# second-state/qwen3_asr_rs

Measured on NVIDIA H100. Metric: real-time factor (audio-sec/wall-sec) Qwen3-ASR-0.6B 30s clips, higher is better.
Workload: dtype f32 (bf16 weights, fp32-exact activations)

## Files before the change

### qwen3_asr_rs_b200/csrc/decode_mega.cu

```cuda
#include "mega_common.cuh"

namespace asrb {

namespace mega {

struct Params {
    const DecLayerW* layers;
    const bf16* lm_head;
    const bf16* embed;
    const float* final_norm;
    const float* rope_cos; const float* rope_sin;
    float eps;
    int L, H, QD, KVD, I, V, nq, nkv, group;
    float* x;
    float* kcache; float* vcache; size_t cache_layer_stride; int max_ctx;
    int nsplit;
    float* part_val; int* part_idx;
    int* pos; int* done; int* next_id; int* ids_out; int* n_out; int max_new;
    unsigned* bar;
    uint2* qkv_ll; uint2* part_ll;
    uint32_t* sx;
    long long* dbg;
    float* part_sum;
    float* lp_out;
    float* eos_lp;
    float* tk_part_val; int* tk_part_idx;
    int* tk_ids; float* tk_lp;
    int* tk_eos_ids; float* tk_eos_lp;
    const SampleParams* smp;
    int row;
    float* part_max; float* part_sel;
    uint32_t* rep_bits;
    int rep_words;
    const RepParams* rep;
};

static_assert(KV_KEYS * HD * 4 == SLOT_BYTES, "K / V tiles travel through the weight ring: one tile per slot");

template <int K>
__device__ __forceinline__ void load_xr(const float* xs, float (&xr)[K / 32], int lane) {
    const int sw = ((lane >> 2) & 1) * 4;
#pragma unroll
    for (int c = 0; c < K / 256; ++c) {
        const float4 a = *reinterpret_cast<const float4*>(xs + (c * 32 + lane) * 8 + sw);
        const float4 b = *reinterpret_cast<const float4*>(xs + (c * 32 + lane) * 8 + 4 - sw);
        xr[c * 8 + 0] = a.x; xr[c * 8 + 1] = a.y; xr[c * 8 + 2] = a.z; xr[c * 8 + 3] = a.w;
        xr[c * 8 + 4] = b.x; xr[c * 8 + 5] = b.y; xr[c * 8 + 6] = b.z; xr[c * 8 + 7] = b.w;
    }
}
// ... 78 lines not shown
        d0 = fmaf(bf16_lo(wd.F), X0, d0); d1 = fmaf(bf16_hi(wd.F), X1, d1);
        ROW4_STEP(x, xr[c * 8 + 0], xr[c * 8 + 1])
        ROW4_STEP(y, xr[c * 8 + 2], xr[c * 8 + 3])
        ROW4_STEP(z, xr[c * 8 + 4], xr[c * 8 + 5])
        ROW4_STEP(w, xr[c * 8 + 6], xr[c * 8 + 7])
#undef ROW4_STEP
    }
    const float ra = a0 + a1, rb = b0 + b1, rc = c0 + c1, rd = d0 + d1;
    const bool h16 = lane & 16, h8 = lane & 8;
    float k0 = (h16 ? rc : ra) + __shfl_xor_sync(0xffffffffu, h16 ? ra : rc, 16);
    float k1 = (h16 ? rd : rb) + __shfl_xor_sync(0xffffffffu, h16 ? rb : rd, 16);
    float keep = (h8 ? k1 : k0) + __shfl_xor_sync(0xffffffffu, h8 ? k0 : k1, 8);
#pragma unroll
    for (int o = 4; o > 0; o >>= 1) keep += __shfl_xor_sync(0xffffffffu, keep, o);
    return keep;
}

__device__ __forceinline__ float warp_reduce8(const float (&a)[8], int lane) {
    const bool h16 = lane & 16, h8 = lane & 8, h4 = lane & 4;
    float k[4];
#pragma unroll
    for (int i = 0; i < 4; ++i) k[i] = (h16 ? a[4 + i] : a[i]) + __shfl_xor_sync(0xffffffffu, h16 ? a[i] : a[4 + i], 16);
    float m0 = (h8 ? k[2] : k[0]) + __shfl_xor_sync(0xffffffffu, h8 ? k[0] : k[2], 8);
    float m1 = (h8 ? k[3] : k[1]) + __shfl_xor_sync(0xffffffffu, h8 ? k[1] : k[3], 8);
    float v = (h4 ? m1 : m0) + __shfl_xor_sync(0xffffffffu, h4 ? m0 : m1, 4);
    v += __shfl_xor_sync(0xffffffffu, v, 2);
    v += __shfl_xor_sync(0xffffffffu, v, 1);
    return v;
}

// ... 321 lines not shown
    ring.slots = smem;
    ring.nslot = NS;
    float* xs = reinterpret_cast<float*>(smem + (size_t)NS * SLOT_BYTES);
    float* xres = xs + XS_FLOATS;
    float* pbuf = xres + XRES_MAX;
    float* ropes = pbuf + 2 * PARAM_FLOATS;
    DecLayerW* ltab = reinterpret_cast<DecLayerW*>(ropes + 128);
    uint64_t* bars = reinterpret_cast<uint64_t*>(ltab + MAX_LAYERS);
    ring.full = bars; ring.empty = bars + NSLOT_MAX;
    uint64_t* p_full = bars + 2 * NSLOT_MAX; uint64_t* p_empty = p_full + 2;
    float* red = reinterpret_cast<float*>(bars + 2 * NSLOT_MAX + 4);
    int* ired = reinterpret_cast<int*>(red + 64);
    float* part = reinterpret_cast<float*>(ired + 64);
    const int tid = threadIdx.x, lane = tid & 31, warp = tid >> 5;
    const bool is_producer = warp == NCONS_WARPS;

    if (__ldcg(p.done) != 0) return;

    if (tid == 0) {
        for (int i = 0; i < NS; ++i) { mbar_init(&ring.full[i], 1); mbar_init(&ring.empty[i], NCONS_WARPS); }
        for (int i = 0; i < 2; ++i) { mbar_init(&p_full[i], 1); mbar_init(&p_empty[i], NCONS_WARPS); }
        asm volatile("fence.mbarrier_init.release.cluster;" ::: "memory");
    }
    const int pos = __ldcg(p.pos);
    {
        const uint2* src = reinterpret_cast<const uint2*>(p.layers);
        uint2* dst = reinterpret_cast<uint2*>(ltab);
        for (int i = tid; i < p.L * (int)(sizeof(DecLayerW) / 8); i += NTHREADS) dst[i] = src[i];
        if (tid < 64) ropes[tid] = p.rope_cos[(size_t)pos * 64 + tid];
        else if (tid < 128) ropes[tid] = p.rope_sin[(size_t)pos * 64 + tid - 64];
// ... 48 lines not shown
                        bulk_g2s(pb, p.final_norm, H * 4, &p_full[l & 1]);
                        break;
                    }
                }
                const DecLayerW w = ltab[l];
                issue_slice(make_slice(w.wqkv, QD + 2 * p.KVD, H, 1));
                if (n_old > 0) {
                    const size_t off = (size_t)l * p.cache_layer_stride + kv_row;
                    issue(p.kcache + off, (uint32_t)n_old * HD * 4);
                    issue(p.vcache + off, (uint32_t)n_old * HD * 4);
                }
                issue_slice(make_slice(w.wo, H, QD, 1));
                issue_slice(make_slice(w.wgu, 2 * I, H, 2));
                issue_slice(make_slice(w.wdown, H, I, 1));
            }
            issue_slice(make_slice(p.lm_head, p.V, H, 1));
        }
        return;
    }

    long long* dbg_row = nullptr; int dbg_i = 0;
    if (p.dbg && (blockIdx.x == 0 || blockIdx.x == gridDim.x - 1)) dbg_row = p.dbg + (blockIdx.x == 0 ? 0 : DBG_SLOTS);
    MEGA_MARK();
    const int half = HD / 2;
    const float* cs = ropes;
    const float* sn = ropes + half;
    const unsigned G = gridDim.x;
    RepBits rb{};
    if constexpr (REP) {
        const Slice sl = make_slice(nullptr, p.V, H, 1);
        uint32_t* hist = p.rep_bits + (size_t)blockIdx.x * 2 * p.rep_words;
// ... 272 lines not shown
        cons_sync();
        if (lane == 0) mbar_arrive(&p_empty[l & 1]);
    }
    float nrf;
    {
        const float ss = sx_gather<H>(sx_cur + (size_t)(p.L - 1) * SXL + H, xs);
        mbar_wait(&p_full[p.L & 1], (p.L >> 1) & 1);
        nrf = norm_scale(ss, H, p.eps, red);
    }
    static_assert(!(SAMPLE && TOPK), "sampling is never combined with the candidate lists");
    static_assert(4 * NCONS_WARPS <= 62, "per-warp records must fit red / ired");
    constexpr bool SLP = SAMPLE && LOGPROB;
    Draw dr{};
    float smx = -INFINITY, ssel = 0.f;
    if constexpr (SAMPLE) dr = make_draw(p.smp, __ldcg(p.n_out), p.row);
    consume<H, ME_ARGMAX, LOGPROB, TOPK, SAMPLE, REP>(make_slice(p.lm_head, p.V, H, 1), ring, q, xs, nullptr, 0u, nullptr, best_v, best_i,
                                                      best_s, pbuf + (p.L & 1) * PARAM_FLOATS, nrf, nullptr, &tk, &dr, &smx, &ssel, &rb);
    MEGA_MARK();
#pragma unroll
    for (int o = 8; o <= 16; o <<= 1) {
        if constexpr (SAMPLE) {
            sample_merge_xor<LOGPROB>(o, best_v, best_i, best_s, smx, ssel);
        } else {
            const float ov = __shfl_xor_sync(0xffffffffu, best_v, o); const int oi = __shfl_xor_sync(0xffffffffu, best_i, o);
            if constexpr (LOGPROB) best_s = lse_merge(best_v, best_s, ov, __shfl_xor_sync(0xffffffffu, best_s, o));
            if (ov > best_v || (ov == best_v && oi < best_i)) { best_v = ov; best_i = oi; }
            if constexpr (TOPK) tk_merge_xor(tk, o);
        }
    }
    cons_sync();
    float* tkv = xs; int* tki = reinterpret_cast<int*>(xs + NCONS_WARPS * TK_MAX);
    if (lane == 0) { red[warp] = best_v; ired[warp] = best_i; if constexpr (LOGPROB) red[NCONS_WARPS + warp] = best_s; }
// ... 10 lines not shown
            float M = -INFINITY;
            for (int wq = 0; wq < NCONS_WARPS; ++wq) M = fmaxf(M, red[2 * NCONS_WARPS + wq]);
            float sum = 0.f;
            for (int wq = 0; wq < NCONS_WARPS; ++wq) sum += lse_rescale(red[NCONS_WARPS + wq], red[2 * NCONS_WARPS + wq], M);
            p.part_sum[blockIdx.x] = sum; p.part_max[blockIdx.x] = M; p.part_sel[blockIdx.x] = red[3 * NCONS_WARPS + ws];
        }
        else if constexpr (LOGPROB) {
            float sum = 0.f;
            for (int wq = 0; wq < NCONS_WARPS; ++wq) sum += lse_rescale(red[NCONS_WARPS + wq], red[wq], v);
            p.part_sum[blockIdx.x] = sum;
        }
        if constexpr (TOPK) {
            for (int wq = 1; wq < NCONS_WARPS; ++wq) tk_merge_from(tk, tkv + wq * TK_MAX, tki + wq * TK_MAX, false);
            tk_store(tk, p.tk_part_val + (size_t)blockIdx.x * TK_MAX, p.tk_part_idx + (size_t)blockIdx.x * TK_MAX);
        }
        __threadfence();
        unsigned t = atomicAdd(p.bar, 1u);
        is_last = (t == G - 1);
    }
    cons_sync();
    if (!is_last) return;
    __threadfence();
    {
        float v = -INFINITY; int idx = 0x7fffffff;
        int rec = 0; float mloc = -INFINITY;
        for (int i = tid; i < (int)G; i += NCONS) {
            float pv = __ldcg(p.part_val + i); int pi = __ldcg(p.part_idx + i);
            if (pv > v || (pv == v && pi < idx)) { v = pv; idx = pi; if constexpr (SLP) rec = i; }
            if constexpr (SLP) mloc = fmaxf(mloc, __ldcg(p.part_max + i));
        }
// ... 40 lines not shown
                if (red[wq] > v || (red[wq] == v && ired[wq] < idx)) { v = red[wq]; idx = ired[wq]; if constexpr (SLP) rec = ired[NCONS_WARPS + wq]; }
            int tok = idx;
            if constexpr (SLP) lp = (__ldcg(p.part_sel + rec) - M) + lp;
            const int n = *p.n_out;
            if constexpr (LOGPROB) {
                if (tok == 151643 || tok == 151645) *p.eos_lp = lp;
                else if (n < p.max_new) p.lp_out[n] = lp;
            }
            if constexpr (TOPK) {
                if (tok == 151643 || tok == 151645) tk_write(tk, lp, p.tk_eos_ids, p.tk_eos_lp);
                else if (n < p.max_new) tk_write(tk, lp, p.tk_ids + (size_t)n * TK_MAX, p.tk_lp + (size_t)n * TK_MAX);
            }
            if (tok == 151643 || tok == 151645 || n >= p.max_new) { *p.done = 1; *p.next_id = -1; tok = -1; }
            else { p.ids_out[n] = tok; *p.n_out = n + 1; *p.pos = pos + 1; *p.next_id = tok; }
            tok_s = tok;
            p.bar[0] = 0;
            p.bar[1] = p.bar[1] + 1;
            p.bar[3] = p.bar[3] + 1;
        }
        cons_sync();
        const int tok = tok_s;
        if (tok >= 0) {
            const bf16* e = p.embed + (size_t)tok * H;
            for (int i = tid; i < H; i += NCONS) p.x[i] = __bfloat162float(e[i]);
        }
    }
}

}

// ... 11 lines not shown
    return c.hidden_size == H && c.num_attention_heads * c.head_dim == QD && c.intermediate_size == I;
}

bool decode_mega_supported(const Model& m, int B, int ctx) {
    const int max_ctx = ctx;
    const asrb_dims& c = m.d.c;
    if (B < 1 || c.head_dim != 128) return false;
    const int group = c.num_attention_heads / c.num_key_value_heads;
    if (group + 2 > mega::NCONS_WARPS) return false;
    if ((size_t)(group * 128 + 256 + group * mega::KV_KEYS + 8 + mega::NCONS_WARPS * 2 * 128 + mega::NCONS_WARPS * 4 + 8) > (size_t)mega_xs_floats(c.intermediate_size)) return false;
    if (m.ctx->smem_optin < mega_smem_bytes(c.hidden_size, c.intermediate_size, mega_nslot(c))) return false;
    if ((c.hidden_size + m.ctx->sm_count - 1) / m.ctx->sm_count + 1 > mega::XRES_MAX) return false;
    if (c.num_hidden_layers > 32) return false;
    if ((max_ctx + mega::KV_KEYS - 1) / mega::KV_KEYS > mega::MAX_SPLITS) return false;
    if (((max_ctx + mega::KV_KEYS - 1) / mega::KV_KEYS) * c.num_key_value_heads > m.ctx->sm_count) return false;
    return dims_match<1024, 2048, 3072>(c) || dims_match<2048, 2048, 6144>(c) || dims_match<256, 512, 512>(c);
}

size_t decode_mega_part_floats(const Model& m) {
    const asrb_dims& c = m.d.c;
    const int group = c.num_attention_heads / c.num_key_value_heads;
    const size_t words = (size_t)m.d.qkv_dim + (size_t)m.ctx->sm_count * group * mega::PSTRIDE + 64;
    return 2 * words + 64;
}
size_t decode_mega_sx_bytes(const Model& m) {
    const asrb_dims& c = m.d.c;
    return 2 * (size_t)c.num_hidden_layers * (2 * (size_t)c.hidden_size + m.d.q_dim + c.intermediate_size) * sizeof(uint32_t);
}

template <bool LP, bool TK, bool SM, bool RP>
// ... 3 lines not shown
    return (const void*)mega::decode_step_kernel<256, 512, 512, 6, LP, TK, SM, RP>;
}
template <bool RP>
static const void* step_fn(const DecodeBufs& b, const asrb_dims& c) {
    if (b.sample) return b.logprobs ? step_fn_dims<true, false, true, RP>(c) : step_fn_dims<false, false, true, RP>(c);
    if (b.topk) return step_fn_dims<true, true, false, RP>(c);
    if (b.logprobs) return step_fn_dims<true, false, false, RP>(c);
    return step_fn_dims<false, false, false, RP>(c);
}

void launch_decode_step_mega(const Model& m, const DecodeBufs& b, int B, float* kcache, float* vcache,
                             size_t cache_layer_stride, size_t cache_seq_stride, int max_ctx, int ctx_now, const MegaBufs& mb,
                             cudaStream_t st, int64_t* launches) {
    ASRB_REQUIRE(decode_mega_supported(m, B, ctx_now), ASRB_ERR_STATE, "fused decode step not supported for this model/batch/context");
    ASRB_REQUIRE(m.d_dec_layers && mb.bar && mb.part && mb.sx_seq, ASRB_ERR_STATE, "fused decode step buffers missing");
    const asrb_dims& c = m.d.c;
    const int G = m.ctx->sm_count;
    const int group = c.num_attention_heads / c.num_key_value_heads;
    const int nsplit = std::min(mega::MAX_SPLITS, std::min(G / c.num_key_value_heads, (max_ctx + mega::KV_KEYS - 1) / mega::KV_KEYS));
    const size_t smem = mega_smem_bytes(c.hidden_size, c.intermediate_size, mega_nslot(c));
    const void* fn = b.rep ? step_fn<true>(b, c) : step_fn<false>(b, c);
    ASRB_CUDA_CHECK(cudaFuncSetAttribute(fn, cudaFuncAttributeMaxDynamicSharedMemorySize, (int)smem));
    for (int sb = 0; sb < B; ++sb) {
        mega::Params p{};
        p.layers = m.d_dec_layers; p.lm_head = m.lm_head; p.embed = m.embed; p.final_norm = m.final_norm_sw;
        p.rope_cos = m.rope_cos; p.rope_sin = m.rope_sin; p.eps = (float)c.rms_norm_eps;
        p.L = c.num_hidden_layers; p.H = c.hidden_size; p.QD = m.d.q_dim; p.KVD = m.d.kv_dim; p.I = c.intermediate_size;
        p.V = c.vocab_size; p.nq = c.num_attention_heads; p.nkv = c.num_key_value_heads; p.group = group;
        p.x = b.x + (size_t)sb * c.hidden_size;
        p.kcache = kcache + (size_t)sb * cache_seq_stride; p.vcache = vcache + (size_t)sb * cache_seq_stride;
// ... 7 lines not shown
        p.part_ll = w;
        p.sx = mb.sx_seq;
        p.dbg = mb.dbg;
        g_last_dbg = mb.dbg;
        if (b.logprobs) { p.part_sum = b.part_sum; p.lp_out = b.lp_out + (size_t)sb * b.max_new; p.eos_lp = b.eos_lp + sb; }
        if (b.topk) {
            p.tk_part_val = b.tk_part_val; p.tk_part_idx = b.tk_part_idx;
            p.tk_ids = b.tk_ids + (size_t)sb * b.max_new * TK_MAX; p.tk_lp = b.tk_lp + (size_t)sb * b.max_new * TK_MAX;
            p.tk_eos_ids = b.tk_eos_ids + (size_t)sb * TK_MAX; p.tk_eos_lp = b.tk_eos_lp + (size_t)sb * TK_MAX;
        }
        if (b.sample) {
            p.smp = b.smp; p.row = sb;
            if (b.logprobs) { p.part_max = b.part_max; p.part_sel = b.part_sel; }
        }
        if (b.rep) { p.rep_bits = b.rep_mask; p.rep_words = rep_cta_words(c, G); p.rep = b.rep_params; }
        if (mb.steps_issued && ++*mb.steps_issued >= 0xFFFF00u) {
            ASRB_CUDA_CHECK(cudaMemsetAsync(mb.part, 0, mb.part_bytes, st));
            const unsigned one = 1;
            ASRB_CUDA_CHECK(cudaMemcpyAsync(mb.bar + 1, &one, sizeof(one), cudaMemcpyHostToDevice, st));
            *mb.steps_issued = 1;
        }
        void* args[] = {(void*)&p};
        ASRB_CUDA_CHECK(cudaLaunchCooperativeKernel(fn, dim3(G), dim3(mega::NTHREADS), args, smem, st));
        if (launches) *launches += 1;
    }
}

int decode_mega_debug_timeline(long long* out, int cap) {
    if (!g_last_dbg || cap < 2 * mega::DBG_SLOTS) return 0;
    cudaDeviceSynchronize();
// ... 7 lines not shown
```

### qwen3_asr_rs_b200/csrc/internal.h

```cpp
#pragma once
#include <atomic>
#include <map>
#include <string>
#include <vector>
#include "../../include/asr_b200.h"
#include "common.cuh"

namespace asrb {

struct Dims {
    asrb_dims c;
    int enc_hd;
    int chunk_frames;
    int chunks_per_window;
    int conv_h[4];
    int conv_w[4];
    int tok_per_chunk;
    int cpad;
    int feat;
    int q_dim, kv_dim, qkv_dim;
    void derive();
};
void validate_dims(const asrb_dims& d);
inline int conv_out_len(int l) { return (l - 1) / 2 + 1; }
// ... 33 lines not shown
    float *mel_fb = nullptr, *dft_cos = nullptr, *dft_sin = nullptr, *hann = nullptr, *dft_tw = nullptr;
    int* mel_krange = nullptr;
    float *conv1_w = nullptr, *conv1_b = nullptr, *conv2_b = nullptr, *conv3_b = nullptr, *conv_out_b = nullptr;
    bf16 *conv2_w = nullptr, *conv3_w = nullptr, *conv_out_w = nullptr;
    float* pos_emb = nullptr;
    std::vector<EncLayerW> enc;
    float *lnpost_w = nullptr, *lnpost_b = nullptr, *proj1_b = nullptr, *proj2_b = nullptr;
    bf16 *proj1 = nullptr, *proj2 = nullptr;
    bf16 *embed = nullptr, *lm_head = nullptr;
    std::vector<DecLayerW> dec;
    float* final_norm = nullptr;
    DecLayerW* d_dec_layers = nullptr;
    float* final_norm_sw = nullptr;
    DecLayerW* d_dec_layers_b = nullptr;
    bf16* lm_head_b = nullptr;
    float *rope_cos = nullptr, *rope_sin = nullptr;
    int rope_max_pos = 0;

    ~Model();
};

enum { A_PLAIN = 0, A_CONV = 1 };
struct GemmA {
    int mode = A_PLAIN;
    const bf16* a = nullptr;
    size_t plane_stride = 0;
    int nplanes = 3;
    int M = 0, K = 0, lda = 0;
    int OH = 0, OW = 0, Hh = 0, Wh = 0, cpad = 0;
};
// ... 90 lines not shown
    float* part_max;
    float* part_sel;
    bool rep;
    const RepParams* rep_params;
    uint32_t* rep_mask;
    int rep_words;
};
void launch_rep_mask(const DecodeBufs& b, int R, cudaStream_t st, int64_t* launches);
inline int rep_cta_words(const asrb_dims& c, int G) { return ((c.vocab_size + G - 1) / G + 31) / 32 + 1; }
void launch_decode_step_phases(const Model& m, const DecodeBufs& b, int B, float* kcache, float* vcache,
                               size_t cache_layer_stride, size_t cache_seq_stride, int max_ctx,
                               bool write_logits, cudaStream_t st, int64_t* launches);
size_t dec_attn_smem_bytes(const Model& m, int max_ctx);
struct MegaBufs { unsigned* bar = nullptr; float* part = nullptr; long long* dbg = nullptr; size_t part_bytes = 0; unsigned* steps_issued = nullptr;
                  uint32_t* sx = nullptr; size_t sx_bytes = 0; int* sx_nb = nullptr;
                  uint32_t* sx_seq = nullptr; };
size_t decode_mega_part_floats(const Model& m);
size_t decode_mega_sx_bytes(const Model& m);
size_t decode_batch_part_floats(const Model& m);
size_t decode_batch_sx_bytes(const Model& m);
bool decode_batch_supported(const Model& m, int B, int ctx);
int decode_mega_dbg_slots();
void launch_greedy(const Model& m, const DecodeBufs& b, int B, cudaStream_t st, int64_t* launches);
void launch_lmhead_argmax(const Model& m, const float* x_rows, const int* d_row_idx, int B,
                          const DecodeBufs& b, bool write_logits, cudaStream_t st, int64_t* launches);

constexpr int BEAM_MAX = 6;
struct BeamUtt {
    int t;
    int done;
    int S;
    int nfin;
// ... 27 lines not shown
```

### qwen3_asr_rs_b200/csrc/model.cu

```cuda
#include <cmath>
#include <cstring>
#include "internal.h"

namespace asrb {

void Dims::derive() {
    enc_hd = c.d_model / c.encoder_attention_heads;
    chunk_frames = 2 * c.n_window;
    chunks_per_window = c.n_window_infer / chunk_frames;
    conv_h[0] = c.num_mel_bins;
    conv_w[0] = chunk_frames;
    for (int i = 1; i < 4; ++i) { conv_h[i] = conv_out_len(conv_h[i - 1]); conv_w[i] = conv_out_len(conv_w[i - 1]); }
    tok_per_chunk = conv_w[3];
    cpad = ((c.downsample_hidden_size + 63) / 64) * 64;
    feat = c.downsample_hidden_size * conv_h[3];
    q_dim = c.num_attention_heads * c.head_dim;
    kv_dim = c.num_key_value_heads * c.head_dim;
    qkv_dim = q_dim + 2 * kv_dim;
}

Model::~Model() {
    for (auto& kv : raw) if (kv.second.dev) cudaFree(kv.second.dev);
    for (void* p : owned) cudaFree(p);
}
// ... 109 lines not shown
    for (size_t i = (size_t)blockIdx.x * blockDim.x + threadIdx.x; i < total; i += (size_t)gridDim.x * blockDim.x) {
        const size_t r = i / chunks; const int cc = (int)(i - r * chunks);
        out[r * chunks + ((cc & ~7) | ((cc ^ (int)(r & 7)) & 7))] = in[i];
    }
}
static bf16* swizzled_rows_copy(Model* m, const bf16* src, size_t n_rows, int K) {
    ASRB_REQUIRE(K % 64 == 0, ASRB_ERR_INVALID, "swizzled copy needs K % 64 == 0");
    bf16* dst = nullptr;
    ASRB_CUDA_CHECK(cudaMalloc(&dst, n_rows * (size_t)K * 2));
    m->owned.push_back(dst);
    swizzle_rows_kernel<<<1184, 256>>>(reinterpret_cast<const uint4*>(src), reinterpret_cast<uint4*>(dst), n_rows, K / 8);
    ASRB_CUDA_CHECK(cudaGetLastError());
    return dst;
}

static float* swizzled_copy(Model* m, const float* dev_src, int n) {
    std::vector<float> h((size_t)n), o((size_t)n);
    ASRB_CUDA_CHECK(cudaMemcpy(h.data(), dev_src, (size_t)n * 4, cudaMemcpyDeviceToHost));
    for (int e = 0; e < n; ++e) { const int k = e >> 2; o[(size_t)((k ^ ((k >> 3) & 1)) << 2) + (e & 3)] = h[e]; }
    float* d = dev_alloc<float>(m, (size_t)n);
    ASRB_CUDA_CHECK(cudaMemcpy(d, o.data(), (size_t)n * 4, cudaMemcpyHostToDevice));
    return d;
}
template <typename T> static T* dev_upload(Model* m, const std::vector<T>& h) {
    T* p = dev_alloc<T>(m, h.size());
    ASRB_CUDA_CHECK(cudaMemcpy(p, h.data(), h.size() * sizeof(T), cudaMemcpyHostToDevice));
    return p;
}
static void drop_raw(Model* m, const std::string& name) {
    auto it = m->raw.find(name);
// ... 200 lines not shown
        ASRB_CUDA_CHECK(cudaMemcpy(m->d_dec_layers, tab.data(), tab.size() * sizeof(DecLayerW), cudaMemcpyHostToDevice));
    }
    if (c.head_dim == 128 && c.num_attention_heads == 2 * c.num_key_value_heads &&
        ((H == 1024 && qd == 2048 && I == 3072) || (H == 256 && qd == 512 && I == 512))) {
        std::vector<DecLayerW> tab = m->dec;
        for (DecLayerW& w : tab) {
            w.wqkv = swizzled_rows_copy(m, w.wqkv, (size_t)d.qkv_dim, (int)H);
            w.wo = swizzled_rows_copy(m, w.wo, (size_t)H, (int)qd);
            w.wgu = swizzled_rows_copy(m, w.wgu, (size_t)2 * I, (int)H);
            w.wdown = swizzled_rows_copy(m, w.wdown, (size_t)H, (int)I);
        }
        m->lm_head_b = swizzled_rows_copy(m, m->lm_head, (size_t)V, (int)H);
        m->d_dec_layers_b = dev_alloc<DecLayerW>(m, tab.size());
        ASRB_CUDA_CHECK(cudaMemcpy(m->d_dec_layers_b, tab.data(), tab.size() * sizeof(DecLayerW), cudaMemcpyHostToDevice));
    }
    build_mel_tables(m);
    build_pos_tables(m);
    ASRB_CUDA_CHECK(cudaDeviceSynchronize());
    m->finalized = true;
}

}
```

### qwen3_asr_rs_b200/csrc/session.cu

```cuda
#include <algorithm>
#include <cerrno>
#include <cmath>
#include <cstdlib>
#include <cstring>
#include <limits>
#include "internal.h"

namespace asrb {

void model_set_tensor(Model* m, const char* name, int dtype, const int64_t* shape, int ndim, const void* host);
void model_finalize(Model* m);
struct IngestState;
IngestState* ingest_state_new();
void ingest_state_free(IngestState* st);
void ingest_pcm(IngestState* st, cudaStream_t stream, const void* const* pcm, const int64_t* n_frames, const int32_t* channels,
                const int32_t* rate, const int32_t* format, int batch, float* d_samples, int64_t max_samples_per_utt,
                int64_t* n_out, int64_t* soff_out);

static const int kPromptHead[9] = {151644, 8948, 198, 151645, 198, 151644, 872, 198, 151669};
static const int kPromptTail[6] = {151670, 151645, 198, 151644, 77091, 198};
static const int kAudioPad = 151676;

struct Session {
    Model* m = nullptr;
// ... 188 lines not shown
                const size_t want = std::min<size_t>({s->mega.sx_bytes, (size_t)maxwin, (size_t)maxpersist});
                if (cudaDeviceSetLimit(cudaLimitPersistingL2CacheSize, want) == cudaSuccess) {
                    cudaStreamAttrValue av{};
                    av.accessPolicyWindow.base_ptr = s->mega.sx; av.accessPolicyWindow.num_bytes = want;
                    av.accessPolicyWindow.hitRatio = 1.0f; av.accessPolicyWindow.hitProp = cudaAccessPropertyPersisting;
                    av.accessPolicyWindow.missProp = cudaAccessPropertyStreaming;
                    if (cudaStreamSetAttribute(s->st, cudaStreamAttributeAccessPolicyWindow, &av) != cudaSuccess) cudaGetLastError();
                } else cudaGetLastError();
            }
        }
        {
            const size_t bytes = decode_mega_sx_bytes(*m);
            s->mega.sx_seq = (uint32_t*)salloc<uint8_t>(s, bytes);
            ASRB_CUDA_CHECK(cudaMemset(s->mega.sx_seq, 0xFF, bytes));
        }
        if (getenv("ASRB_MEGA_DEBUG")) s->mega.dbg = salloc<long long>(s, decode_mega_dbg_slots(), true);
        ASRB_CUDA_CHECK(cudaMallocHost(&s->h_done, Bm * sizeof(int)));
        ASRB_CUDA_CHECK(cudaMallocHost(&s->h_nout, Bm * sizeof(int)));
        ASRB_CUDA_CHECK(cudaMallocHost(&s->h_next, Bm * sizeof(int)));
        ASRB_CUDA_CHECK(cudaMallocHost(&s->h_ids, Bm * max_new * sizeof(int)));
        ASRB_CUDA_CHECK(cudaDeviceSynchronize());
    } catch (...) { delete s; throw; }
    return s;
}

void session_free(Session* s) { delete s; }

static void mel_impl(Session* s, const float* const* samples, const int64_t* n_samples, int batch, const int64_t* view_off,
                     int64_t* n_frames_out) {
    ASRB_REQUIRE(batch >= 1 && batch <= s->max_batch, ASRB_ERR_INVALID, "batch exceeds session capacity");
// ... 714 lines not shown
        const int n = std::min(s->h_nout[b], max_new_tokens);
        for (int i = 0; i < max_new_tokens; ++i)
            for (int j = 0; j < k; ++j) {
                const size_t o = ((size_t)b * max_new_tokens + i) * k + j, src = ((size_t)b * s->max_new + i) * TK_MAX + j;
                ids_out[o] = i < n ? ids[src] : -1;
                lp_out[o] = i < n ? lp[src] : nan;
            }
        for (int j = 0; j < k; ++j) {
            if (eos_ids_out) eos_ids_out[(size_t)b * k + j] = eids[(size_t)b * TK_MAX + j];
            if (eos_lp_out) eos_lp_out[(size_t)b * k + j] = elp[(size_t)b * TK_MAX + j];
        }
    }
}

void session_stats(Session* s, int64_t* out, int n) {
    const int64_t v[5] = {s->n_batch_steps, s->n_mega_steps, s->n_phase_steps, g_gemm_simt_fallbacks.load(), g_gemm_tc_launches.load()};
    for (int i = 0; i < n && i < 5; ++i) out[i] = v[i];
}

void session_last_nbest(Session* s, int max_new_tokens, int k, int32_t* ids_out, int32_t* lens_out, float* sum_out,
                        float* score_out, int32_t* eos_out) {
    ASRB_REQUIRE(s->stage >= 3 && s->nbest_valid, ASRB_ERR_STATE, "last_nbest: the last run was not a beam run");
    ASRB_REQUIRE(max_new_tokens >= 1, ASRB_ERR_INVALID, "max_new_tokens must be >= 1");
    ASRB_REQUIRE(k >= 1 && k <= s->run_k, ASRB_ERR_INVALID, "k must be in [1, beam_size of the last run]");
    ASRB_CUDA_CHECK(cudaSetDevice(s->m->ctx->device));
    const int B = s->B, K = s->run_k;
    std::vector<int32_t> ids((size_t)B * K * s->max_new);
    ASRB_CUDA_CHECK(cudaMemcpyAsync(ids.data(), s->beam.nb_ids, ids.size() * sizeof(int32_t), cudaMemcpyDeviceToHost, s->st));
    ASRB_CUDA_CHECK(cudaStreamSynchronize(s->st));
    for (int b = 0; b < B; ++b)
        for (int j = 0; j < k; ++j) {
            const size_t o = (size_t)b * K + j, d = (size_t)b * k + j;
// ... 131 lines not shown
```

### qwen3_asr_rs_b200/inference.py

```python
from __future__ import annotations

import ctypes as C
import math
import os
from dataclasses import dataclass
from typing import Callable, Dict, List, Optional, Sequence, Tuple, Union

import numpy as np

from . import _lib
from .config import AsrConfig

EOS_TOKEN_IDS = (151643, 151645)
MAX_NEW_TOKENS = 4096
MEL_SAMPLE_RATE = 16000

_DT = {"float32": 0, "bfloat16": 1, "float16": 2}


def _dims_struct(cfg: AsrConfig) -> _lib.AsrbDims:
    a, t = cfg.audio, cfg.text
    d = _lib.AsrbDims()
    for k in ("d_model", "encoder_layers", "encoder_attention_heads", "encoder_ffn_dim", "num_mel_bins",
              "max_source_positions", "n_window", "n_window_infer", "downsample_hidden_size", "output_dim"):
# ... 302 lines not shown
        except Exception:
            pass

    def set_option(self, key: str, value: str) -> None:
        self._options[key] = value
        if self._session is not None:
            _lib.check(self._lib.asrb_session_set_option(self._session, key.encode(), value.encode()))

    def device_ids(self):
        ids, lens = C.c_void_p(), C.c_void_p()
        stride, batch = C.c_int(), C.c_int()
        _lib.check(self._lib.asrb_session_device_ids(self._session, C.byref(ids), C.byref(lens), C.byref(stride), C.byref(batch)))
        return ids.value, lens.value, stride.value, batch.value

    def stats(self) -> Dict[str, int]:
        out = (C.c_int64 * 5)()
        if self._session is None:
            return {}
        _lib.check(self._lib.asrb_session_stats(self._session, out, 5))
        return dict(zip(("decode_batch_steps", "decode_fused_steps", "decode_phase_steps", "gemm_simt_fallbacks",
                         "gemm_tc_launches"), [int(v) for v in out]))

    def _ensure_session(self, batch: int, max_samples: int, max_lang: int, max_new: int, max_context: int = 0):
        cap = self._cap
        if cap is None or batch > cap[0] or max_samples > cap[1] or max_lang > cap[2] or max_new > cap[3] \
                or max_context > cap[4]:
            if self._session is not None:
                _lib.check(self._lib.asrb_session_free(self._session))
                self._session, self._cap = None, None
            new_cap = (max(batch, cap[0] if cap else 0), max(max_samples, cap[1] if cap else 0),
                       max(max_lang, cap[2] if cap else 0), max(max_new, cap[3] if cap else 0),
                       max(max_context, cap[4] if cap else 0))
            s = C.c_void_p()
            _lib.check(self._lib.asrb_session_create_ex(self._model, new_cap[0], new_cap[1], new_cap[2], new_cap[4],
                                                        new_cap[3], C.byref(s)))
            self._session, self._cap = s, new_cap
# ... 543 lines not shown
```

Before: 314.5.

## Screen greedy lm_head argmax with int8 weights and exact rescoring of candidates

```diff
diff --git a/lmhead_candidates.py b/lmhead_candidates.py
--- /dev/null
+++ b/lmhead_candidates.py
@@ -0,0 +1,64 @@
+import argparse
+import json
+
+import numpy as np
+
+from oracle import oracle as O
+from qwen3_asr_rs_b200 import synth
+
+
+def main():
+    ap = argparse.ArgumentParser()
+    ap.add_argument("--model", default="0p6b", choices=["0p6b", "1p7b"])
+    ap.add_argument("--new-tokens", type=int, default=128)
+    ap.add_argument("--ctas", type=int, default=132)
+    args = ap.parse_args()
+    cfg = O.cfg_0p6b() if args.model == "0p6b" else O.cfg_1p7b()
+    xs = []
+
+    class Capture(O.OracleModel):
+        def decoder_forward(self, hidden, cos, sin, cache, mask, last_only=False, from_row=0):
+            x = hidden
+            for i in range(self.cfg.text.num_hidden_layers):
+                x = self.decoder_layer(x, i, cos, sin, cache, mask)
+            x = O.rms_norm(x, self.w["thinker.model.norm.weight"], self.cfg.text.rms_norm_eps)
+            xs.append(x[0, -1].double().numpy())
+            return x[:, -1:, :].matmul(self.lm_head_weight().t())
+
+    m = Capture(cfg, synth.make_weights(cfg, 1))
+    ids = O.transcribe_ids(m, synth.make_clip(0), max_new_tokens=args.new_tokens, lm_head_all_rows=False).ids
+    steps = xs[1:len(ids)]
+    W = m.lm_head_weight().float().numpy().astype(np.float64)
+    V, K = W.shape
+    u = 2.0 ** -24
+    n = K // 64 + 6
+    gamma = lambda k: k * u / (1 - k * u)
+    s = (np.abs(W).max(1) / 127).astype(np.float32).astype(np.float64)
+    q = np.clip(np.rint(W / np.where(s > 0, s, 1)[:, None]), -127, 127)
+    nq = np.linalg.norm(q, axis=1)
+    C = np.linalg.norm(W - s[:, None] * q, axis=1) + gamma(n) * np.linalg.norm(W, axis=1) + gamma(n + 1) * s * nq
+    G = args.ctas
+    bounds = [((c * V) // G, ((c + 1) * V) // G) for c in range(G)]
+    counts = {"a": [], "b": []}
+    for x in steps:
+        nx = np.linalg.norm(x) * (1 + 2 ** -12)
+        a, B = s * (q @ x), nx * C
+        sx = np.abs(x).max() / 127
+        qx = np.rint(x / sx)
+        ab, Bb = s * sx * (q @ qx), B + np.linalg.norm(x - sx * qx) * (1 + 2 ** -12) * s * nq
+        for form, (aa, bb) in (("a", (a, B)), ("b", (ab, Bb))):
+            row = []
+            for r0, r1 in bounds:
+                T = np.max(aa[r0:r1] - bb[r0:r1])
+                row.append(int(np.count_nonzero(aa[r0:r1] + bb[r0:r1] >= T)))
+            counts[form].append(row)
+    out = {"model": args.model, "tokens": len(ids), "steps": len(steps), "ctas": G, "rows_per_cta": V // G}
+    for form, c in counts.items():
+        c = np.array(c)
+        out[form] = {"per_cta_mean": round(float(c.mean()), 2), "per_cta_max": int(c.max()),
+                     "per_step_mean": round(float(c.sum(1).mean()), 1), "per_step_max": int(c.sum(1).max())}
+    print(json.dumps(out))
+
+
+if __name__ == "__main__":
+    main()
diff --git a/qwen3_asr_rs_b200/csrc/decode_mega.cu b/qwen3_asr_rs_b200/csrc/decode_mega.cu
--- a/qwen3_asr_rs_b200/csrc/decode_mega.cu
+++ b/qwen3_asr_rs_b200/csrc/decode_mega.cu
@@ -1,3 +1,5 @@
+#include <cfloat>
+#include <climits>
 #include "mega_common.cuh"
 
 namespace asrb {
@@ -33,6 +35,9 @@
     uint32_t* rep_bits;
     int rep_words;
     const RepParams* rep;
+    const int8_t* lm_head_q;
+    const float2* lm_head_sc;
+    unsigned long long* hq_stats;
 };
 
 static_assert(KV_KEYS * HD * 4 == SLOT_BYTES, "K / V tiles travel through the weight ring: one tile per slot");
@@ -141,6 +146,129 @@
 #pragma unroll
     for (int o = 4; o > 0; o >>= 1) keep += __shfl_xor_sync(0xffffffffu, keep, o);
     return keep;
+}
+
+__device__ __forceinline__ void i8x4_f32(uint32_t w, float (&f)[4]) {
+    const uint32_t u = w ^ 0x80808080u;
+    f[0] = __uint_as_float(__byte_perm(u, 0x4B000000u, 0x7540)) - 8388736.f;
+    f[1] = __uint_as_float(__byte_perm(u, 0x4B000000u, 0x7541)) - 8388736.f;
+    f[2] = __uint_as_float(__byte_perm(u, 0x4B000000u, 0x7542)) - 8388736.f;
+    f[3] = __uint_as_float(__byte_perm(u, 0x4B000000u, 0x7543)) - 8388736.f;
+}
+template <int K>
+__device__ __forceinline__ float row_dot4_q(const uint2* w0, const uint2* w1, const uint2* w2, const uint2* w3,
+                                            const float (&xr)[K / 32], int lane) {
+    float a0 = 0.f, a1 = 0.f, b0 = 0.f, b1 = 0.f, c0 = 0.f, c1 = 0.f, d0 = 0.f, d1 = 0.f;
+#pragma unroll
+    for (int c = 0; c < K / 256; ++c) {
+        const uint2 wa = w0[c * 32 + lane], wb = w1[c * 32 + lane], wc = w2[c * 32 + lane], wd = w3[c * 32 + lane];
+        float fa[4], fb[4], fc[4], fd[4];
+#define ROWQ_STEP(F, O)                                                                                               \
+        i8x4_f32(wa.F, fa); i8x4_f32(wb.F, fb); i8x4_f32(wc.F, fc); i8x4_f32(wd.F, fd);                               \
+        a0 = fmaf(fa[0], xr[c * 8 + O], a0); a1 = fmaf(fa[1], xr[c * 8 + O + 1], a1);                                 \
+        b0 = fmaf(fb[0], xr[c * 8 + O], b0); b1 = fmaf(fb[1], xr[c * 8 + O + 1], b1);                                 \
+        c0 = fmaf(fc[0], xr[c * 8 + O], c0); c1 = fmaf(fc[1], xr[c * 8 + O + 1], c1);                                 \
+        d0 = fmaf(fd[0], xr[c * 8 + O], d0); d1 = fmaf(fd[1], xr[c * 8 + O + 1], d1);                                 \
+        a0 = fmaf(fa[2], xr[c * 8 + O + 2], a0); a1 = fmaf(fa[3], xr[c * 8 + O + 3], a1);                             \
+        b0 = fmaf(fb[2], xr[c * 8 + O + 2], b0); b1 = fmaf(fb[3], xr[c * 8 + O + 3], b1);                             \
+        c0 = fmaf(fc[2], xr[c * 8 + O + 2], c0); c1 = fmaf(fc[3], xr[c * 8 + O + 3], c1);                             \
+        d0 = fmaf(fd[2], xr[c * 8 + O + 2], d0); d1 = fmaf(fd[3], xr[c * 8 + O + 3], d1);
+        ROWQ_STEP(x, 0)
+        ROWQ_STEP(y, 4)
+#undef ROWQ_STEP
+    }
+    const float ra = a0 + a1, rb = b0 + b1, rc = c0 + c1, rd = d0 + d1;
+    const bool h16 = lane & 16, h8 = lane & 8;
+    float k0 = (h16 ? rc : ra) + __shfl_xor_sync(0xffffffffu, h16 ? ra : rc, 16);
+    float k1 = (h16 ? rd : rb) + __shfl_xor_sync(0xffffffffu, h16 ? rb : rd, 16);
+    float keep = (h8 ? k1 : k0) + __shfl_xor_sync(0xffffffffu, h8 ? k0 : k1, 8);
+#pragma unroll
+    for (int o = 4; o > 0; o >>= 1) keep += __shfl_xor_sync(0xffffffffu, keep, o);
+    return keep;
+}
+__device__ __forceinline__ int f32_ord(float f) { const int i = __float_as_int(f); return i >= 0 ? i : -(i & 0x7fffffff); }
+
+static constexpr int HQ_CAP = 256;
+
+template <int K>
+__device__ __forceinline__ void consume_head_q(const Slice& s, const Ring& ring, uint32_t& q, float* xs, const float2* hsc,
+                                               float& best_v, int& best_i, const float* norm_w, float norm_r) {
+    static_assert(SLOT_BYTES / K == 16 || (SLOT_BYTES / K) % 32 == 0, "a turn is 32 rows: one slot, or a pair of 16-row slots");
+    const int lane = threadIdx.x & 31, warp = threadIdx.x >> 5;
+    constexpr int NU = K / 8;
+    float xr[K / 32];
+    load_xr_norm<K>(xs, norm_w, norm_r, xr, lane);
+    float ss = 0.f;
+#pragma unroll
+    for (int i = 0; i < K / 32; ++i) ss = fmaf(xr[i], xr[i], ss);
+    ss = warp_sum(ss);
+    const float nx = __fmul_ru(sqrtf(ss), 1.f + 0x1p-12f);
+    int* const st = reinterpret_cast<int*>(xs);
+    int2* const cl = reinterpret_cast<int2*>(xs + 4);
+    cons_sync();
+    if (threadIdx.x == 0) { st[0] = INT_MIN; st[1] = 0; st[2] = !(ss >= 0x1p-60f); st[3] = 0; }
+    cons_sync();
+    const int j = lane >> 3;
+    auto fetch = [&](int t) { return __ldg(hsc + min(s.r0 + 32 * t + 4 * warp + j, s.r1 - 1)); };
+    float2 win = fetch(lane & 7), nxt = fetch(8 + (lane & 7));
+    int t = 0;
+    for (int r = s.r0; r < s.r1;) {
+        const int rowsA = min(s.rpc, s.r1 - r);
+        const uint32_t slotA = q % ring.nslot;
+        mbar_wait(&ring.full[slotA], (q / ring.nslot) & 1);
+        const bool pair = s.rpc < 32 && r + rowsA < s.r1;
+        const int rowsB = pair ? min(s.rpc, s.r1 - r - rowsA) : 0;
+        const uint32_t slotB = (q + 1) % ring.nslot;
+        if (pair) mbar_wait(&ring.full[slotB], ((q + 1) / ring.nslot) & 1);
+        const uint2* baseA = reinterpret_cast<const uint2*>(ring.slots + (size_t)slotA * SLOT_BYTES);
+        const uint2* baseB = reinterpret_cast<const uint2*>(ring.slots + (size_t)slotB * SLOT_BYTES);
+        const int R = rowsA + rowsB;
+        for (int i0 = 4 * warp; i0 < R; i0 += 4 * NCONS_WARPS, ++t) {
+            const int nv = min(4, R - i0);
+            const uint2* rp[4];
+#pragma unroll
+            for (int i = 0; i < 4; ++i) {
+                const int ri = i0 + (i < nv ? i : 0);
+                rp[i] = ri < rowsA ? baseA + (size_t)ri * NU : baseB + (size_t)(ri - rowsA) * NU;
+            }
+            const float g = row_dot4_q<K>(rp[0], rp[1], rp[2], rp[3], xr, lane);
+            const int src = (lane & 24) | (t & 7);
+            const float sr = __shfl_sync(0xffffffffu, win.x, src), cr = __shfl_sync(0xffffffffu, win.y, src);
+            if ((t & 7) == 7) { win = nxt; nxt = fetch(t + 9 + (lane & 7)); }
+            const float a = g * sr;
+            const float b = __fadd_ru(__fmul_ru(nx, cr), 0x1p-100f);
+            const float lo = __fsub_rd(a, b), hi = __fadd_ru(a, b);
+            const bool mine = (lane & 7) == 0 && j < nv;
+            const bool finite = fabsf(lo) <= FLT_MAX && fabsf(hi) <= FLT_MAX;
+            if (mine && !finite) st[2] = 1;
+            int tw = mine && finite ? f32_ord(lo) : INT_MIN;
+            tw = max(tw, __shfl_xor_sync(0xffffffffu, tw, 8));
+            tw = max(tw, __shfl_xor_sync(0xffffffffu, tw, 16));
+            int T = 0;
+            if (lane == 0) T = max(atomicMax(st, tw), tw);
+            T = __shfl_sync(0xffffffffu, T, 0);
+            if (mine && finite && f32_ord(hi) >= T) {
+                const int k = atomicAdd(st + 1, 1);
+                if (k < HQ_CAP) cl[k] = make_int2(r + i0 + j, f32_ord(hi));
+            }
+        }
+        __syncwarp();
+        if (lane == 0) { mbar_arrive(&ring.empty[slotA]); if (pair) mbar_arrive(&ring.empty[slotB]); }
+        r += R; q += pair ? 2 : 1;
+    }
+    cons_sync();
+    const int T = st[0], n = st[1];
+    const bool full = n > HQ_CAP || st[2] != 0;
+    const int cnt = full ? s.r1 - s.r0 : n;
+    int done = 0;
+    for (int k = warp; k < cnt; k += NCONS_WARPS) {
+        int row = s.r0 + k;
+        if (!full) { const int2 e = cl[k]; if (e.y < T) continue; row = e.x; }
+        const float v = row_dot<K>(reinterpret_cast<const uint4*>(s.W + (size_t)row * K), xr, lane);
+        if (v > best_v || (v == best_v && row < best_i)) { best_v = v; best_i = row; }
+        ++done;
+    }
+    if (lane == 0) atomicAdd(st + 3, done);
 }
 
 __device__ __forceinline__ float warp_reduce8(const float (&a)[8], int lane) {
@@ -492,6 +620,7 @@
     float* part = reinterpret_cast<float*>(ired + 64);
     const int tid = threadIdx.x, lane = tid & 31, warp = tid >> 5;
     const bool is_producer = warp == NCONS_WARPS;
+    constexpr bool HEADQ = !LOGPROB && !TOPK && !SAMPLE && !REP;
 
     if (__ldcg(p.done) != 0) return;
 
@@ -570,7 +699,13 @@
                 issue_slice(make_slice(w.wgu, 2 * I, H, 2));
                 issue_slice(make_slice(w.wdown, H, I, 1));
             }
-            issue_slice(make_slice(p.lm_head, p.V, H, 1));
+            if constexpr (HEADQ) {
+                const Slice sl = make_slice(nullptr, p.V, H, 1);
+                constexpr int RQ = SLOT_BYTES / H;
+                for (int r = sl.r0; r < sl.r1; r += RQ) issue(p.lm_head_q + (size_t)r * H, (uint32_t)min(RQ, sl.r1 - r) * H);
+            } else {
+                issue_slice(make_slice(p.lm_head, p.V, H, 1));
+            }
         }
         return;
     }
@@ -873,8 +1008,15 @@
     Draw dr{};
     float smx = -INFINITY, ssel = 0.f;
     if constexpr (SAMPLE) dr = make_draw(p.smp, __ldcg(p.n_out), p.row);
-    consume<H, ME_ARGMAX, LOGPROB, TOPK, SAMPLE, REP>(make_slice(p.lm_head, p.V, H, 1), ring, q, xs, nullptr, 0u, nullptr, best_v, best_i,
-                                                      best_s, pbuf + (p.L & 1) * PARAM_FLOATS, nrf, nullptr, &tk, &dr, &smx, &ssel, &rb);
+    if constexpr (HEADQ) {
+        Slice sl = make_slice(p.lm_head, p.V, H, 1);
+        sl.rpc = SLOT_BYTES / H;
+        consume_head_q<H>(sl, ring, q, xs, p.lm_head_sc, best_v, best_i, pbuf + (p.L & 1) * PARAM_FLOATS, nrf);
+    } else {
+        consume<H, ME_ARGMAX, LOGPROB, TOPK, SAMPLE, REP>(make_slice(p.lm_head, p.V, H, 1), ring, q, xs, nullptr, 0u, nullptr, best_v,
+                                                          best_i, best_s, pbuf + (p.L & 1) * PARAM_FLOATS, nrf, nullptr, &tk, &dr, &smx,
+                                                          &ssel, &rb);
+    }
     MEGA_MARK();
 #pragma unroll
     for (int o = 8; o <= 16; o <<= 1) {
@@ -915,6 +1057,11 @@
             for (int wq = 1; wq < NCONS_WARPS; ++wq) tk_merge_from(tk, tkv + wq * TK_MAX, tki + wq * TK_MAX, false);
             tk_store(tk, p.tk_part_val + (size_t)blockIdx.x * TK_MAX, p.tk_part_idx + (size_t)blockIdx.x * TK_MAX);
         }
+        if constexpr (HEADQ) {
+            const int* st = reinterpret_cast<const int*>(xs);
+            atomicAdd(p.hq_stats, (unsigned long long)st[3]);
+            if (st[1] > HQ_CAP || st[2] != 0) atomicAdd(p.hq_stats + 3, 1ull);
+        }
         __threadfence();
         unsigned t = atomicAdd(p.bar, 1u);
         is_last = (t == G - 1);
@@ -985,6 +1132,11 @@
             if (tok == 151643 || tok == 151645 || n >= p.max_new) { *p.done = 1; *p.next_id = -1; tok = -1; }
             else { p.ids_out[n] = tok; *p.n_out = n + 1; *p.pos = pos + 1; *p.next_id = tok; }
             tok_s = tok;
+            if constexpr (HEADQ) {
+                const unsigned long long nr = __ldcg(p.hq_stats);
+                p.hq_stats[0] = 0; p.hq_stats[1] = __ldcg(p.hq_stats + 1) + nr;
+                if (nr > __ldcg(p.hq_stats + 2)) p.hq_stats[2] = nr;
+            }
             p.bar[0] = 0;
             p.bar[1] = p.bar[1] + 1;
             p.bar[3] = p.bar[3] + 1;
@@ -1026,6 +1178,9 @@
     if (c.num_hidden_layers > 32) return false;
     if ((max_ctx + mega::KV_KEYS - 1) / mega::KV_KEYS > mega::MAX_SPLITS) return false;
     if (((max_ctx + mega::KV_KEYS - 1) / mega::KV_KEYS) * c.num_key_value_heads > m.ctx->sm_count) return false;
+    return decode_mega_dims(c);
+}
+bool decode_mega_dims(const asrb_dims& c) {
     return dims_match<1024, 2048, 3072>(c) || dims_match<2048, 2048, 6144>(c) || dims_match<256, 512, 512>(c);
 }
 
@@ -1059,6 +1214,8 @@
                              cudaStream_t st, int64_t* launches) {
     ASRB_REQUIRE(decode_mega_supported(m, B, ctx_now), ASRB_ERR_STATE, "fused decode step not supported for this model/batch/context");
     ASRB_REQUIRE(m.d_dec_layers && mb.bar && mb.part && mb.sx_seq, ASRB_ERR_STATE, "fused decode step buffers missing");
+    const bool greedy = !b.logprobs && !b.topk && !b.sample && !b.rep;
+    ASRB_REQUIRE(!greedy || (m.lm_head_q && m.lm_head_sc && mb.hq_stats), ASRB_ERR_STATE, "fused decode step: int8 lm_head copy missing");
     const asrb_dims& c = m.d.c;
     const int G = m.ctx->sm_count;
     const int group = c.num_attention_heads / c.num_key_value_heads;
@@ -1096,6 +1253,7 @@
             if (b.logprobs) { p.part_max = b.part_max; p.part_sel = b.part_sel; }
         }
         if (b.rep) { p.rep_bits = b.rep_mask; p.rep_words = rep_cta_words(c, G); p.rep = b.rep_params; }
+        p.lm_head_q = m.lm_head_q; p.lm_head_sc = m.lm_head_sc; p.hq_stats = mb.hq_stats;
         if (mb.steps_issued && ++*mb.steps_issued >= 0xFFFF00u) {
             ASRB_CUDA_CHECK(cudaMemsetAsync(mb.part, 0, mb.part_bytes, st));
             const unsigned one = 1;
diff --git a/qwen3_asr_rs_b200/csrc/internal.h b/qwen3_asr_rs_b200/csrc/internal.h
--- a/qwen3_asr_rs_b200/csrc/internal.h
+++ b/qwen3_asr_rs_b200/csrc/internal.h
@@ -71,6 +71,8 @@
     float* final_norm_sw = nullptr;
     DecLayerW* d_dec_layers_b = nullptr;
     bf16* lm_head_b = nullptr;
+    int8_t* lm_head_q = nullptr;
+    float2* lm_head_sc = nullptr;
     float *rope_cos = nullptr, *rope_sin = nullptr;
     int rope_max_pos = 0;
 
@@ -191,8 +193,10 @@
 size_t dec_attn_smem_bytes(const Model& m, int max_ctx);
 struct MegaBufs { unsigned* bar = nullptr; float* part = nullptr; long long* dbg = nullptr; size_t part_bytes = 0; unsigned* steps_issued = nullptr;
                   uint32_t* sx = nullptr; size_t sx_bytes = 0; int* sx_nb = nullptr;
-                  uint32_t* sx_seq = nullptr; };
+                  uint32_t* sx_seq = nullptr;
+                  unsigned long long* hq_stats = nullptr; };
 size_t decode_mega_part_floats(const Model& m);
+bool decode_mega_dims(const asrb_dims& c);
 size_t decode_mega_sx_bytes(const Model& m);
 size_t decode_batch_part_floats(const Model& m);
 size_t decode_batch_sx_bytes(const Model& m);
diff --git a/qwen3_asr_rs_b200/csrc/model.cu b/qwen3_asr_rs_b200/csrc/model.cu
--- a/qwen3_asr_rs_b200/csrc/model.cu
+++ b/qwen3_asr_rs_b200/csrc/model.cu
@@ -147,6 +147,32 @@
     return dst;
 }
 
+__global__ void quantize_head_kernel(const bf16* __restrict__ w, int8_t* __restrict__ q, float2* __restrict__ sc, int V, int K,
+                                     double gn, double gn1) {
+    const int lane = threadIdx.x & 31, row = blockIdx.x * (blockDim.x >> 5) + (threadIdx.x >> 5);
+    if (row >= V) return;
+    const bf16* wr = w + (size_t)row * K;
+    float amax = 0.f;
+    for (int k = lane; k < K; k += 32) amax = fmaxf(amax, fabsf(__bfloat162float(wr[k])));
+    for (int o = 16; o > 0; o >>= 1) amax = fmaxf(amax, __shfl_xor_sync(0xffffffffu, amax, o));
+    const float s = amax / 127.f;
+    double r2 = 0.0, w2 = 0.0, q2 = 0.0;
+    for (int k = lane; k < K; k += 32) {
+        const float v = __bfloat162float(wr[k]);
+        const float qf = s > 0.f ? fminf(fmaxf(rintf(v / s), -127.f), 127.f) : 0.f;
+        q[(size_t)row * K + k] = (int8_t)qf;
+        const double d = (double)v - (double)s * (double)qf;
+        r2 += d * d; w2 += (double)v * (double)v; q2 += (double)qf * (double)qf;
+    }
+    for (int o = 16; o > 0; o >>= 1) {
+        r2 += __shfl_xor_sync(0xffffffffu, r2, o); w2 += __shfl_xor_sync(0xffffffffu, w2, o); q2 += __shfl_xor_sync(0xffffffffu, q2, o);
+    }
+    if (lane == 0) {
+        const double C = (sqrt(r2) + gn * sqrt(w2) + gn1 * (double)s * sqrt(q2)) * (1.0 + 1e-9);
+        sc[row] = make_float2(s, __double2float_ru(C));
+    }
+}
+
 static float* swizzled_copy(Model* m, const float* dev_src, int n) {
     std::vector<float> h((size_t)n), o((size_t)n);
     ASRB_CUDA_CHECK(cudaMemcpy(h.data(), dev_src, (size_t)n * 4, cudaMemcpyDeviceToHost));
@@ -377,6 +403,15 @@
         m->d_dec_layers_b = dev_alloc<DecLayerW>(m, tab.size());
         ASRB_CUDA_CHECK(cudaMemcpy(m->d_dec_layers_b, tab.data(), tab.size() * sizeof(DecLayerW), cudaMemcpyHostToDevice));
     }
+    if (decode_mega_dims(c)) {
+        const int n = (int)H / 64 + 6;
+        const double u = std::ldexp(1.0, -24);
+        auto gamma = [&](int k) { return k * u / (1.0 - k * u); };
+        m->lm_head_q = dev_alloc<int8_t>(m, (size_t)V * H);
+        m->lm_head_sc = dev_alloc<float2>(m, (size_t)V);
+        quantize_head_kernel<<<(unsigned)((V + 7) / 8), 256>>>(m->lm_head, m->lm_head_q, m->lm_head_sc, (int)V, (int)H, gamma(n), gamma(n + 1));
+        ASRB_CUDA_CHECK(cudaGetLastError());
+    }
     build_mel_tables(m);
     build_pos_tables(m);
     ASRB_CUDA_CHECK(cudaDeviceSynchronize());
diff --git a/qwen3_asr_rs_b200/csrc/session.cu b/qwen3_asr_rs_b200/csrc/session.cu
--- a/qwen3_asr_rs_b200/csrc/session.cu
+++ b/qwen3_asr_rs_b200/csrc/session.cu
@@ -226,6 +226,7 @@
             s->mega.sx_seq = (uint32_t*)salloc<uint8_t>(s, bytes);
             ASRB_CUDA_CHECK(cudaMemset(s->mega.sx_seq, 0xFF, bytes));
         }
+        s->mega.hq_stats = salloc<unsigned long long>(s, 4, true);
         if (getenv("ASRB_MEGA_DEBUG")) s->mega.dbg = salloc<long long>(s, decode_mega_dbg_slots(), true);
         ASRB_CUDA_CHECK(cudaMallocHost(&s->h_done, Bm * sizeof(int)));
         ASRB_CUDA_CHECK(cudaMallocHost(&s->h_nout, Bm * sizeof(int)));
@@ -970,8 +971,15 @@
 }
 
 void session_stats(Session* s, int64_t* out, int n) {
-    const int64_t v[5] = {s->n_batch_steps, s->n_mega_steps, s->n_phase_steps, g_gemm_simt_fallbacks.load(), g_gemm_tc_launches.load()};
-    for (int i = 0; i < n && i < 5; ++i) out[i] = v[i];
+    unsigned long long hq[4] = {0, 0, 0, 0};
+    if (n > 5 && s->mega.hq_stats) {
+        ASRB_CUDA_CHECK(cudaSetDevice(s->m->ctx->device));
+        ASRB_CUDA_CHECK(cudaMemcpyAsync(hq, s->mega.hq_stats, sizeof(hq), cudaMemcpyDeviceToHost, s->st));
+        ASRB_CUDA_CHECK(cudaStreamSynchronize(s->st));
+    }
+    const int64_t v[8] = {s->n_batch_steps, s->n_mega_steps, s->n_phase_steps, g_gemm_simt_fallbacks.load(), g_gemm_tc_launches.load(),
+                          (int64_t)hq[1], (int64_t)hq[2], (int64_t)hq[3]};
+    for (int i = 0; i < n && i < 8; ++i) out[i] = v[i];
 }
 
 void session_last_nbest(Session* s, int max_new_tokens, int k, int32_t* ids_out, int32_t* lens_out, float* sum_out,
diff --git a/qwen3_asr_rs_b200/inference.py b/qwen3_asr_rs_b200/inference.py
--- a/qwen3_asr_rs_b200/inference.py
+++ b/qwen3_asr_rs_b200/inference.py
@@ -340,12 +340,13 @@
         return ids.value, lens.value, stride.value, batch.value
 
     def stats(self) -> Dict[str, int]:
-        out = (C.c_int64 * 5)()
+        out = (C.c_int64 * 8)()
         if self._session is None:
             return {}
-        _lib.check(self._lib.asrb_session_stats(self._session, out, 5))
+        _lib.check(self._lib.asrb_session_stats(self._session, out, 8))
         return dict(zip(("decode_batch_steps", "decode_fused_steps", "decode_phase_steps", "gemm_simt_fallbacks",
-                         "gemm_tc_launches"), [int(v) for v in out]))
+                         "gemm_tc_launches", "lmhead_rows_recomputed", "lmhead_step_max_recomputed",
+                         "lmhead_full_fallbacks"), [int(v) for v in out]))
 
     def _ensure_session(self, batch: int, max_samples: int, max_lang: int, max_new: int, max_context: int = 0):
         cap = self._cap
```

Result: faster. 336.7, median of 6 (+7.1%).
